# annalam/seqkit

Hardware: AMD Instinct MI355X
Metric: M reads/s demultiplex (150bp, 96 barcodes) at 1/8 GPUs; % HBM roofline (higher is better)
Workload: dtype u8

## Files before the change

### seqkit_amd/build.py

```python
from __future__ import annotations

import os
import shutil
import subprocess
import sys

ROOT = os.path.dirname(os.path.abspath(__file__))
REPO = os.path.dirname(ROOT)
CSRC = os.path.join(ROOT, "csrc")
LIBDIR = os.path.join(ROOT, "lib")
BINDIR = os.path.join(ROOT, "bin")
LIB_PATH = os.path.join(LIBDIR, "libseqkit_hip.so")

HIP_SOURCES = ["sk_kernels.hip", "sk_census.hip", "sk_inflate.hip", "sk_deflate.hip", "sk_bamtext.hip", "sk_bamwrite.hip", "sk_bamminimize.hip", "sk_bammarkdup.hip", "sk_bamsubsample.hip", "sk_bammerge.hip", "sk_bamcoverage.hip", "sk_bampair.hip", "sk_bamtarget.hip", "sk_capi.hip", "sk_bamfile.cpp", "sk_bamfile_reads.cpp", "sk_bamfile_out.cpp", "sk_bamfile_coverage.cpp", "sk_lut.cpp"]
HIP_DEPS = HIP_SOURCES + ["sk_internal.h", "sk_lut.h", "sk_bamblock.h", "sk_bamfmt.h", "sk_bamfile.h", "sk_passmem.h", os.path.join(REPO, "include", "seqkit_hip.h")]
HIP_FLAGS = ["--offload-arch=gfx950", "-O3", "-std=c++17", "-fPIC", "-shared", "-Wall", "-Wno-unused-function"]


def library_inputs_digest() -> str:
    import hashlib
    h = hashlib.sha256()
    h.update(" ".join(HIP_FLAGS).encode())
    for d in HIP_DEPS:
        p = d if os.path.isabs(d) else os.path.join(CSRC, d)
        with open(p, "rb") as f:
            h.update(os.path.basename(p).encode() + b"\0" + f.read())
    return h.hexdigest()[:16]


def _hipcc() -> str:
    for cand in (os.environ.get("HIPCC"), shutil.which("hipcc"), "/opt/rocm/bin/hipcc"):
        if cand and os.path.exists(cand):
            return cand
    raise RuntimeError("hipcc not found: the gfx950 library cannot be built")


def _stale(target: str, deps: list[str]) -> bool:
    if not os.path.exists(target):
        return True
    t = os.path.getmtime(target)
    for d in deps:
        p = d if os.path.isabs(d) else os.path.join(CSRC, d)
        if os.path.exists(p) and os.path.getmtime(p) > t:
            return True
    return False


def _run(cmd: list[str], cwd: str) -> None:
    r = subprocess.run(cmd, cwd=cwd, stdout=subprocess.PIPE, stderr=subprocess.STDOUT, text=True)
    if r.returncode != 0:
        sys.stderr.write(r.stdout)
        raise RuntimeError("build failed: " + " ".join(cmd))


def build_library(force: bool = False, verbose: bool = False) -> str:
    os.makedirs(LIBDIR, exist_ok=True)
    if force or _stale(LIB_PATH, HIP_DEPS):
        cmd = [_hipcc()] + HIP_FLAGS + ["-o", LIB_PATH] + HIP_SOURCES + ["-ldl", "-lz", "-pthread"]
        if verbose:
            cmd.append("-Rpass-analysis=kernel-resource-usage")
        _run(cmd, CSRC)
    return LIB_PATH


def build_hosts(force: bool = False) -> list[str]:
    os.makedirs(BINDIR, exist_ok=True)
    out = []
    for name, srcs, libs in (("fasta", ["host_common.cpp", "host_inflate.cpp", "fasta_main.cpp", "fasta_text.cpp"], ["-lz", "-ldl"]),
                             ("sam", ["host_common.cpp", "host_inflate.cpp", "sam_main.cpp"], ["-lz", "-ldl"])):
        if not all(os.path.exists(os.path.join(CSRC, s)) for s in srcs):
            continue
        target = os.path.join(BINDIR, name)
        deps = srcs + ["host_common.h", "sam_pairing.h", "sk_bamfmt.h", os.path.join(REPO, "include", "seqkit_hip.h"), LIB_PATH]
        if force or _stale(target, deps):
            cmd = ["g++", "-O2", "-std=c++17", "-Wall", "-Wextra", "-pthread", "-I", os.path.join(REPO, "include"),
                   "-o", target] + srcs + ["-L", LIBDIR, "-lseqkit_hip", "-Wl,-rpath,$ORIGIN/../lib"] + libs
            _run(cmd, CSRC)
        out.append(target)
    return out


def build_all(force: bool = False) -> None:
    build_library(force=force)
    build_hosts(force=force)


if __name__ == "__main__":
    build_all(force="--force" in sys.argv)
    print(LIB_PATH)
```

### seqkit_amd/csrc/sk_kernels.hip

```cpp
#include "sk_internal.h"

#include <cstdlib>
#include <mutex>
#include <vector>

namespace sk {

#ifndef SK_STRAGGLER_FROM
#define SK_STRAGGLER_FROM 6
#endif
#ifndef SK_STRAGGLER_ROWS
#define SK_STRAGGLER_ROWS 8
#endif
#ifndef SK_STRAGGLER_LEFT
#define SK_STRAGGLER_LEFT 6
#endif

typedef uint32_t u32;
typedef __attribute__((ext_vector_type(4))) uint32_t u32x4;
typedef __attribute__((ext_vector_type(2))) uint32_t u32x2;

typedef const __attribute__((address_space(4))) uint32_t *const_u32_ptr;

constexpr u32 kLo7 = 0x7f7f7f7fu;
constexpr u32 kHi1 = 0x80808080u;

QualConsts make_qual_consts(int m)
{
	QualConsts q{};
	q.min_baseq = m;
	q.cl2 = 0; q.c72 = 0;
	if (m == 0) { q.mode = 0; return q; }
	int t2;
	if (33 + m <= 255) { q.mode = 1; t2 = 33 + m; }
	else if (33 + m == 256) { q.mode = 3; t2 = 1; }
	else { q.mode = 4; t2 = 33 + m - 256; }
	int c2 = 256 - t2;
	q.cl2 = (u32)(c2 & 0x7f) * 0x01010101u;
	q.c72 = (c2 & 0x80) ? kHi1 : 0u;
	if (q.mode == 1 && !(c2 & 0x80)) q.mode = 2;
	return q;
}

template <int MODE>
__device__ __forceinline__ u32 lowq_flags(u32 q, u32 ql, u32 t1, u32 cl2)
{
	if (MODE == 0) return 0u;
	u32 g1 = q | t1;
	if (MODE == 3) return g1;
	u32 t2 = ql + cl2;
	u32 g2 = (MODE == 2) ? (q & t2) : (q | t2);
	if (MODE == 4) return g1 | ~g2;
	return g1 & ~g2;
}

__device__ __forceinline__ u32 mask_select(u32 s, u32 F)
{
	u32 sel = ((F >> 5) & 0x04040404u) | 0x03020100u;
	return __builtin_amdgcn_perm(0x4e4e4e4eu, s, sel);
}

__device__ __forceinline__ u32 sub33(u32 q, u32 t1) { return t1 ^ (~q & kHi1); }

template <int MODE>
__device__ __forceinline__ void mask_dword4(const u32x4 &q, const u32x4 &s, u32 cl2, u32x4 &out, u32x4 &vq)
{
#pragma unroll
	for (int i = 0; i < 4; i++) {
		u32 ql = q[i] & kLo7;
		u32 t1 = ql + 0x5f5f5f5fu;
		vq[i] = sub33(q[i], t1);
		out[i] = mask_select(s[i], lowq_flags<MODE>(q[i], ql, t1, cl2));
	}
}

#ifndef SK_NT
#define SK_NT 3
#endif
__device__ __forceinline__ u32x4 stream_load(const uint8_t *p)
{
#if SK_NT & 1
	return __builtin_nontemporal_load(reinterpret_cast<const u32x4 *>(p));
#else
	return *reinterpret_cast<const u32x4 *>(p);
#endif
}
__device__ __forceinline__ void stream_store(uint8_t *p, const u32x4 &v)
{
#if SK_NT & 2
	__builtin_nontemporal_store(v, reinterpret_cast<u32x4 *>(p));
#else
	*reinterpret_cast<u32x4 *>(p) = v;
#endif
}

__device__ __forceinline__ u32x4 load_tail(const uint8_t *p, int valid)
{
	u32x4 v = {0u, 0u, 0u, 0u};
	for (int b = 0; b < valid; b++) v[b >> 2] |= (u32)p[b] << (8 * (b & 3));
	return v;
}
__device__ __forceinline__ void store_tail(uint8_t *p, const u32x4 &v, int valid)
{
	for (int b = 0; b < valid; b++) p[b] = (uint8_t)(v[b >> 2] >> (8 * (b & 3)));
}

template <int MODE>
__global__ __launch_bounds__(256) void mask_flat_kernel(const uint8_t *__restrict__ seq, const uint8_t *__restrict__ qual,
                                                        uint8_t *__restrict__ out, int64_t bytes, u32 cl2)
{
#ifndef SK_MASK_UNROLL
#define SK_MASK_UNROLL 4
#endif
	constexpr int kUnroll = SK_MASK_UNROLL;
	const int64_t nchunk = (bytes + 15) >> 4;
	const int64_t nspan = (nchunk + 256 * kUnroll - 1) / (256 * kUnroll);
	for (int64_t sp = blockIdx.x; sp < nspan; sp += gridDim.x) {
		const int64_t c0 = sp * (256 * kUnroll) + (threadIdx.x >> 6) * (64 * kUnroll) + (threadIdx.x & 63);
		if ((sp + 1) * (256 * kUnroll) * 16 <= bytes) {
			u32x4 q[kUnroll], sv[kUnroll];
#pragma unroll
			for (int k = 0; k < kUnroll; k++) {
				const int64_t off = (c0 + k * 64) << 4;
				q[k] = stream_load(qual + off);
				sv[k] = stream_load(seq + off);
			}
#pragma unroll
			for (int k = 0; k < kUnroll; k++) {
				u32x4 o, vq;
				mask_dword4<MODE>(q[k], sv[k], cl2, o, vq);
				stream_store(out + ((c0 + k * 64) << 4), o);
			}
		} else {
			for (int k = 0; k < kUnroll; k++) {
				const int64_t c = c0 + k * 64;
				if (c >= nchunk) break;
				const int64_t off = c << 4;
				u32x4 q, s, o, vq;
				if (off + 16 <= bytes) {
					q = *reinterpret_cast<const u32x4 *>(qual + off);
					s = *reinterpret_cast<const u32x4 *>(seq + off);
					mask_dword4<MODE>(q, s, cl2, o, vq);
					*reinterpret_cast<u32x4 *>(out + off) = o;
				} else {
					int valid = (int)(bytes - off);
					q = load_tail(qual + off, valid);
					s = load_tail(seq + off, valid);
					mask_dword4<MODE>(q, s, cl2, o, vq);
					store_tail(out + off, o, valid);
				}
			}
		}
	}
// ... 1934 lines not shown
			u32x4 e4 = {0u, 0u, 0u, 0u}, mt4 = e4, mp4 = e4, tl4 = e4;
			if (a.single_end) e4 = *reinterpret_cast<const u32x4 *>(a.end_pos + r0);
			else {
				mt4 = *reinterpret_cast<const u32x4 *>(a.mtid + r0);
				mp4 = *reinterpret_cast<const u32x4 *>(a.mpos + r0);
				tl4 = *reinterpret_cast<const u32x4 *>(a.tlen + r0);
			}
#pragma unroll
			for (int u = 0; u < kCountIlp; u++) {
				fl[u] = (f2[u >> 1] >> (16 * (u & 1))) & 0xffffu;
				mq[u] = (m4 >> (8 * u)) & 0xffu;
				posv[u] = (int32_t)p4[u]; tidv[u] = (int32_t)t4[u];
				mtidv[u] = (int32_t)mt4[u]; mposv[u] = (int32_t)mp4[u]; tlenv[u] = (int32_t)tl4[u]; endv[u] = (int32_t)e4[u];
			}
		} else {
#pragma unroll
			for (int u = 0; u < kCountIlp; u++) {
				const int64_t rc = r0 + u < a.n ? r0 + u : r0;
				fl[u] = a.flag[rc]; mq[u] = a.mapq[rc]; posv[u] = a.pos[rc]; tidv[u] = a.tid[rc];
				endv[u] = a.single_end ? a.end_pos[rc] : 0;
				mtidv[u] = a.single_end ? 0 : a.mtid[rc]; mposv[u] = a.single_end ? 0 : a.mpos[rc]; tlenv[u] = a.single_end ? 0 : a.tlen[rc];
			}
		}
		u32 start[kCountIlp], end[kCountIlp];
		int lo[kCountIlp], b[kCountIlp], e[kCountIlp];
#pragma unroll
		for (int u = 0; u < kCountIlp; u++) {
			const u32 f = fl[u];
			bool ok = r0 + u < a.n;
			ok = ok && !(f & (0x4u | 0x400u | 0x100u | 0x800u));
			ok = ok && mq[u] >= a.min_mapq;
			const int32_t pos = posv[u], tid = tidv[u];
			u32 st = (u32)pos, en;
			if (a.single_end) {
				en = (u32)endv[u];
			} else {
				ok = ok && (f & 0x1u) && !(f & 0x8u);
				ok = ok && tid == mtidv[u];
				const int32_t mpos = mposv[u];
				ok = ok && !(pos > mpos || (pos == mpos && !(f & 0x40u)));
				const int32_t tl = tlenv[u];
				const u32 ins = tl < 0 ? 0u - (u32)tl : (u32)tl;
				ok = ok && ins >= 20u;
				en = st + ins;
			}
			ok = ok && en - st <= a.max_frag_len;
			if (a.center) { st += (en - st) / 2u; en = st + 1u; }
			ok = ok && tid >= 0 && tid < a.n_chr;
			const int tc = ok ? tid : 0;
			lo[u] = a.chr_off[tc];
			b[u] = lo[u];
			e[u] = ok ? a.chr_off[tc + 1] : lo[u];
			start[u] = st;
			end[u] = en;
		}
		int hi_prev = -1;
#pragma unroll
		for (int u = 0; u < kCountIlp; u++) {
			const int hi = e[u];
			if (u > 0 && lo[u] == lo[u - 1] && hi == hi_prev && hi > lo[u]) b[u] = region_gallop(a.rstart, lo[u], hi, b[u - 1], end[u]);
			else b[u] = region_lower_bound(a.rstart, lo[u], hi, end[u]);
			hi_prev = hi;
		}
#pragma unroll
		for (int u = 0; u < kCountIlp; u++) {
			for (int i = b[u] - 1; i >= lo[u]; i--) {
				if (a.rpmax[i] <= start[u]) break;
				if (a.rend[i] > start[u]) atomicAdd(&a.counts[a.ridx[i]], 1u);
			}
		}
	}
}

hipError_t launch_bam_count(const CountArgs &a, int n_cu, hipStream_t st)
{
	if (a.n <= 0) return hipSuccess;
	const int64_t want = (a.n + 256 * kCountIlp - 1) / (256 * kCountIlp);
	const int grid = (int)(want < (int64_t)n_cu * 8 ? want : (int64_t)n_cu * 8);
	uintptr_t bits = (uintptr_t)a.flag | (uintptr_t)a.mapq | (uintptr_t)a.pos | (uintptr_t)a.tid;
	bits |= a.single_end ? (uintptr_t)a.end_pos : ((uintptr_t)a.mtid | (uintptr_t)a.mpos | (uintptr_t)a.tlen);
	if ((bits & 15u) == 0) bam_count_kernel<true><<<grid, 256, 0, st>>>(a);
	else bam_count_kernel<false><<<grid, 256, 0, st>>>(a);
	return hipGetLastError();
}

__device__ __forceinline__ u32 zero_bytes(u32 x)
{
	return ~(((x & 0x7F7F7F7Fu) + 0x7F7F7F7Fu) | x | 0x7F7F7F7Fu);
}

__device__ __forceinline__ void gc_dword(u32 w, u32 &gc, u32 &non_n)
{
	const u32 up = w & 0xDFDFDFDFu;
	gc += (u32)__popc(zero_bytes(up ^ 0x43434343u) | zero_bytes(up ^ 0x47474747u));
	non_n += 4u - (u32)__popc(zero_bytes(up ^ 0x4E4E4E4Eu));
}

__device__ __forceinline__ void gc_byte(u32 b, u32 &gc, u32 &non_n)
{
	const u32 up = b & 0xDFu;
	gc += (up == 0x43u || up == 0x47u) ? 1u : 0u;
	non_n += (up != 0x4Eu) ? 1u : 0u;
}

__global__ __launch_bounds__(256) void gc_count_kernel(const uint8_t *__restrict__ genome, const int64_t *__restrict__ seg_start,
                                                       const int32_t *__restrict__ seg_len, const int32_t *__restrict__ seg_region, int64_t nseg,
                                                       unsigned long long *__restrict__ out )
{
	const int lane = threadIdx.x & 63;
	const int64_t wave = ((int64_t)blockIdx.x * blockDim.x + threadIdx.x) >> 6, nwaves = ((int64_t)gridDim.x * blockDim.x) >> 6;
	for (int64_t s = wave; s < nseg; s += nwaves) {
		const uint8_t *p = genome + seg_start[s];
		const int n = seg_len[s];
		u32 gc = 0, non_n = 0;
		int head = (int)((16 - ((uintptr_t)p & 15)) & 15);
		if (head > n) head = n;
		if (lane < head) gc_byte(p[lane], gc, non_n);
		const int body = (n - head) & ~15;
		const u32x4 *v = reinterpret_cast<const u32x4 *>(p + head);
		const int nchunk = body >> 4;
		int i = lane;
		for (; i + 192 < nchunk; i += 256) {
			u32x4 w[4];
#pragma unroll
			for (int k = 0; k < 4; k++) w[k] = stream_load(reinterpret_cast<const uint8_t *>(v + i + 64 * k));
#pragma unroll
			for (int k = 0; k < 4; k++) { gc_dword(w[k][0], gc, non_n); gc_dword(w[k][1], gc, non_n); gc_dword(w[k][2], gc, non_n); gc_dword(w[k][3], gc, non_n); }
		}
		for (; i < nchunk; i += 64) {
			const u32x4 w = stream_load(reinterpret_cast<const uint8_t *>(v + i));
			gc_dword(w[0], gc, non_n); gc_dword(w[1], gc, non_n); gc_dword(w[2], gc, non_n); gc_dword(w[3], gc, non_n);
		}
		const int tail0 = head + body;
		if (tail0 + lane < n) gc_byte(p[tail0 + lane], gc, non_n);
		for (int o = 32; o > 0; o >>= 1) { gc += __shfl_xor(gc, o); non_n += __shfl_xor(non_n, o); }
		if (lane == 0) {
			const int r = seg_region[s];
			if (gc) atomicAdd(&out[2 * r], (unsigned long long)gc);
			if (non_n) atomicAdd(&out[2 * r + 1], (unsigned long long)non_n);
		}
	}
}

hipError_t launch_gc_count(const uint8_t *genome, const int64_t *seg_start, const int32_t *seg_len, const int32_t *seg_region, int64_t nseg,
                           unsigned long long *out, int n_cu, hipStream_t st)
{
	if (nseg <= 0) return hipSuccess;
	const int64_t want = (nseg + 3) / 4;
	const int grid = (int)(want < (int64_t)n_cu * 8 ? want : (int64_t)n_cu * 8);
	gc_count_kernel<<<grid, 256, 0, st>>>(genome, seg_start, seg_len, seg_region, nseg, out);
	return hipGetLastError();
}

constexpr u32 kN4 = 0x4E4E4E4Eu;

__device__ __forceinline__ u32 bases_from_codes(u32 nib, bool complement)
{
	const u32 lo = complement ? 0x4E47544Eu : 0x4E43414Eu;
	const u32 hi = complement ? 0x4E4E4E43u : 0x4E4E4E47u;
	const u32 lo8 = complement ? 0x4E4E4E41u : 0x4E4E4E54u;
	const u32 sel = nib & 0x07070707u;
	const u32 r_low = __builtin_amdgcn_perm(hi, lo, sel);
	const u32 r_high = __builtin_amdgcn_perm(kN4, lo8, sel);
	const u32 is_high = ((nib >> 3) & 0x01010101u) * 0xFFu;
	return (r_high & is_high) | (r_low & ~is_high);
}

template <bool SMALL_M>
__device__ __forceinline__ u32 bytes_below(u32 q, u32 m4)
{
	const u32 d = (q | kHi1) - (m4 & ~kHi1);
	const u32 lt = SMALL_M ? (~(q | d) & kHi1) : (((~q & m4) | (~(q ^ m4) & ~d)) & kHi1);
	return (lt >> 7) * 0xFFu;
}

__device__ __forceinline__ u32 spread_nibbles(u32 h)
{
	u32 x = (h | (h << 8)) & 0x00FF00FFu;
	return (x | (x << 4)) & 0x0F0F0F0Fu;
}

#ifndef SK_SEQ_UNROLL
#define SK_SEQ_UNROLL 1
#endif
constexpr int kSeqUnroll = SK_SEQ_UNROLL;
template <bool SMALL_M>
__global__ __launch_bounds__(256) void bam_sequence8_kernel(const uint8_t *__restrict__ seq4, int seq4_stride, const uint8_t *__restrict__ qual,
                                                            int stride, const uint16_t *__restrict__ len, const uint16_t *__restrict__ flag,
                                                            int64_t n, u32 m4, u32 inv_upr, uint8_t *__restrict__ out)
{
	__shared__ u32 row_info[64];
	const int upr = (stride + 7) >> 3;
	const bool half_tail = (stride & 7) != 0;
	const int64_t ntiles = (n + 63) / 64;
	for (int64_t t = blockIdx.x; t < ntiles; t += gridDim.x) {
		const int64_t row0 = t * 64;
		const int rows = (int)((n - row0) < 64 ? (n - row0) : 64);
		__syncthreads();
		if ((int)threadIdx.x < rows) {
			const int64_t r = row0 + threadIdx.x;
			const u32 l = len ? (u32)len[r] : (u32)stride;
			row_info[threadIdx.x] = l | (((u32)flag[r] >> 4) & 1u) << 16;
		}
		__syncthreads();
		const rsrc_t rq = make_rsrc(qual, row0 * (int64_t)stride, rows * stride);
		const rsrc_t rs = make_rsrc(seq4, row0 * (int64_t)seq4_stride, rows * seq4_stride);
		const rsrc_t ro = make_rsrc(out, row0 * (int64_t)stride, rows * stride);
		const u32 total = (u32)rows * (u32)upr;
		for (u32 e = threadIdx.x; e < total; e += blockDim.x * kSeqUnroll) {
			u32 rlv[kSeqUnroll], w0v[kSeqUnroll];
			int jv[kSeqUnroll], s0v[kSeqUnroll];
			bool revv[kSeqUnroll];
			u32x2 w12v[kSeqUnroll], ddv[kSeqUnroll];
#pragma unroll
			for (int u = 0; u < kSeqUnroll; u++) {
				const u32 eu = e + (u32)u * blockDim.x;
				const u32 ec = eu < total ? eu : total - 1;
				const u32 rl = inv_upr ? __umulhi(ec, inv_upr) : ec / (u32)upr;
				const int j = (int)(ec - rl * (u32)upr);
				const u32 info = row_info[rl];
				const int l = (int)(info & 0xFFFFu);
				const bool rev = (info >> 16) != 0u;
				int s0 = rev ? l - 8 - 8 * j : 8 * j;
				if (s0 < -8) s0 = -8;
				const int qrow = (int)rl * stride, qd = s0 >> 2;
				w0v[u] = __builtin_amdgcn_raw_buffer_load_b32(rq, qrow + 4 * (qd < 0 ? 0 : qd), 0, 0);
				w12v[u] = __builtin_amdgcn_raw_buffer_load_b64(rq, qrow + 4 * (qd + 1 < 0 ? 0 : qd + 1), 0, 0);
				const int sd = (s0 >> 1) >> 2;
				ddv[u] = __builtin_amdgcn_raw_buffer_load_b64(rs, (int)rl * seq4_stride + 4 * (sd < 0 ? 0 : sd), 0, 0);
				rlv[u] = rl; jv[u] = j; s0v[u] = s0; revv[u] = rev;
			}
#pragma unroll
			for (int u = 0; u < kSeqUnroll; u++) {
				const int s0 = s0v[u];
				const bool rev = revv[u];
				const int qd = s0 >> 2;
				const u32 sh = (u32)s0 & 3u;
				const u32 w0 = w0v[u], w1 = w12v[u][0], w2 = qd + 1 < 0 ? w12v[u][0] : w12v[u][1];
				const u32 qa = __builtin_amdgcn_alignbyte(w1, w0, sh), qb = __builtin_amdgcn_alignbyte(w2, w1, sh);
				const int a = s0 >> 1, sd = a >> 2;
				const u32 d0 = ddv[u][0], d1 = sd < 0 ? ddv[u][0] : ddv[u][1];
				const u32 b03 = __builtin_amdgcn_alignbyte(d1, d0, (u32)a & 3u);
				const u32 b4 = __builtin_amdgcn_alignbyte(0u, d1, (u32)a & 3u) & 0xFFu;
				const u32 be = __builtin_bswap32(b03);
				const u32 n8 = (s0 & 1) ? ((be << 4) | (b4 >> 4)) : be;
				const u32 c_first = spread_nibbles(n8 >> 16), c_last = spread_nibbles(n8 & 0xFFFFu);
				u32 q_lo, q_hi, n_lo, n_hi;
				if (rev) {
					q_lo = __builtin_amdgcn_perm(0u, qb, 0x00010203u); q_hi = __builtin_amdgcn_perm(0u, qa, 0x00010203u);
					n_lo = c_last; n_hi = c_first;
				} else {
					q_lo = qa; q_hi = qb;
					n_lo = __builtin_amdgcn_perm(0u, c_first, 0x00010203u); n_hi = __builtin_amdgcn_perm(0u, c_last, 0x00010203u);
				}
				const u32 lo_low = bytes_below<SMALL_M>(q_lo, m4), hi_low = bytes_below<SMALL_M>(q_hi, m4);
				u32x2 o;
				o[0] = (kN4 & lo_low) | (bases_from_codes(n_lo, rev) & ~lo_low);
				o[1] = (kN4 & hi_low) | (bases_from_codes(n_hi, rev) & ~hi_low);
				if (e + (u32)u * blockDim.x < total) {
					if (half_tail && jv[u] == upr - 1) __builtin_amdgcn_raw_buffer_store_b32(o[0], ro, (int)rlv[u] * stride + 8 * jv[u], 0, 0);
					else __builtin_amdgcn_raw_buffer_store_b64(o, ro, (int)rlv[u] * stride + 8 * jv[u], 0, 0);
				}
			}
		}
	}
}

#ifndef SK_SEQ_TWO
#define SK_SEQ_TWO 0
#endif
template <bool SMALL_M, int NQ, int ROWS>
__global__ __launch_bounds__(256, ROWS == 64 ? 2 : 4) void bam_sequence_tile_kernel(const uint8_t *__restrict__ seq4, int seq4_stride, const uint8_t *__restrict__ qual,
                                                                   int stride, const uint16_t *__restrict__ len, const uint16_t *__restrict__ flag,
                                                                   int64_t n, u32 m4, u32 inv_upr, uint8_t *__restrict__ out)
{
	constexpr int NS = (NQ + 1) / 2;
	constexpr int kSlot = (NQ + NS) * 1024 + 256;
	constexpr int kMaxU = NQ * 2;
	static_assert(ROWS == 64 || ROWS == 32, "a tile is one or half a row per lane");
	const int lane = threadIdx.x & 63;
	const int wave = __builtin_amdgcn_readfirstlane(threadIdx.x >> 6);
	uint8_t *img = sk_smem + wave * kSlot;
	uint8_t *simg = img + NQ * 1024;
	u32 *info = reinterpret_cast<u32 *>(img + (NQ + NS) * 1024);
	const int upr = (stride + 7) >> 3;
	const bool half_tail = (stride & 4) != 0;
	const int64_t ntiles = (n + ROWS - 1) / ROWS;
	const int64_t tstep = (int64_t)gridDim.x * 4;
	auto fetch = [&](int64_t t, u32x4 (&rq)[NQ], u32x4 (&rs)[NS], u32 &rinfo) {
		const int rows = t < ntiles ? (int)((n - t * ROWS) < ROWS ? (n - t * ROWS) : ROWS) : 0;
		const int64_t row0 = rows ? t * ROWS : 0;
		const rsrc_t dq = make_rsrc(qual, row0 * (int64_t)stride, rows * stride), ds = make_rsrc(seq4, row0 * (int64_t)seq4_stride, (rows * seq4_stride + 3) & ~3);
#pragma unroll
		for (int c = 0; c < NQ; c++) rq[c] = __builtin_amdgcn_raw_buffer_load_b128(dq, c * 1024 + lane * 16, 0, kAuxStream);
#pragma unroll
		for (int c = 0; c < NS; c++) rs[c] = __builtin_amdgcn_raw_buffer_load_b128(ds, c * 1024 + lane * 16, 0, kAuxStream);
		const u32 lv = (u32)(unsigned short)__builtin_amdgcn_raw_buffer_load_b16(make_rsrc(len, row0 * 2, rows * 2), lane * 2, 0, 0);
		const u32 fv = (u32)(unsigned short)__builtin_amdgcn_raw_buffer_load_b16(make_rsrc(flag, row0 * 2, rows * 2), lane * 2, 0, 0);
		rinfo = (len ? lv : (u32)stride) | ((fv >> 4) & 1u) << 16;
	};
	auto process = [&](int64_t t, int ahead, u32x4 (&rq)[NQ], u32x4 (&rs)[NS], u32 &rinfo) {
		const int64_t row0 = t * ROWS;
		const int rows = (int)((n - row0) < ROWS ? (n - row0) : ROWS);
		const u32 units = (u32)(ROWS * upr);
#pragma unroll
		for (int c = 0; c < NQ; c++) *reinterpret_cast<u32x4 *>(img + c * 1024 + lane * 16) = rq[c];
#pragma unroll
		for (int c = 0; c < NS; c++) *reinterpret_cast<u32x4 *>(simg + c * 1024 + lane * 16) = rs[c];
		info[lane] = rinfo;
		wave_lds_fence();
		fetch(t + ahead * tstep, rq, rs, rinfo);
		u32x2 ov[kMaxU];
#pragma unroll
		for (int i = 0; i < kMaxU; i++) {
			ov[i][0] = ov[i][1] = 0u;
			if (64u * (u32)i < units) {
				const u32 ee = (u32)lane + 64u * (u32)i;
				const u32 e = ee < units ? ee : units - 1u;
				const u32 rl = inv_upr ? __umulhi(e, inv_upr) : e / (u32)upr;
				const int j = (int)(e - rl * (u32)upr);
				const u32 inf = info[rl];
				const int l = (int)(inf & 0xFFFFu);
				const bool rev = (inf >> 16) != 0u;
				int s0 = rev ? l - 8 - 8 * j : 8 * j;
				if (s0 < -8) s0 = -8;
				const int qrow = (int)rl * stride, qd = s0 >> 2;
				const u32 *qw = reinterpret_cast<const u32 *>(img + qrow);
				const u32 w0 = qw[qd < 0 ? 0 : qd], w1 = qw[qd + 1 < 0 ? 0 : qd + 1], w2 = qw[qd + 2 < 0 ? 0 : qd + 2];
				const u32 sh = (u32)s0 & 3u;
				const u32 qa = __builtin_amdgcn_alignbyte(w1, w0, sh), qb = __builtin_amdgcn_alignbyte(w2, w1, sh);
				const int a = s0 >> 1, sd = a >> 2;
				const u32 *sw = reinterpret_cast<const u32 *>(simg + (int)rl * seq4_stride);
				const u32 d0 = sw[sd < 0 ? 0 : sd], d1 = sw[sd + 1 < 0 ? 0 : sd + 1];
				const u32 b03 = __builtin_amdgcn_alignbyte(d1, d0, (u32)a & 3u);
				const u32 b4 = __builtin_amdgcn_alignbyte(0u, d1, (u32)a & 3u) & 0xFFu;
				const u32 be = __builtin_bswap32(b03);
				const u32 n8 = (s0 & 1) ? ((be << 4) | (b4 >> 4)) : be;
				const u32 c_first = spread_nibbles(n8 >> 16), c_last = spread_nibbles(n8 & 0xFFFFu);
				u32 q_lo, q_hi, n_lo, n_hi;
				if (rev) {
					q_lo = __builtin_amdgcn_perm(0u, qb, 0x00010203u); q_hi = __builtin_amdgcn_perm(0u, qa, 0x00010203u);
					n_lo = c_last; n_hi = c_first;
				} else {
					q_lo = qa; q_hi = qb;
					n_lo = __builtin_amdgcn_perm(0u, c_first, 0x00010203u); n_hi = __builtin_amdgcn_perm(0u, c_last, 0x00010203u);
				}
				const u32 lo_low = bytes_below<SMALL_M>(q_lo, m4), hi_low = bytes_below<SMALL_M>(q_hi, m4);
				ov[i][0] = (kN4 & lo_low) | (bases_from_codes(n_lo, rev) & ~lo_low);
				ov[i][1] = (kN4 & hi_low) | (bases_from_codes(n_hi, rev) & ~hi_low);
			}
		}
		wave_lds_fence();
		if (!half_tail) {
#pragma unroll
			for (int i = 0; i < kMaxU; i++)
				if ((u32)lane + 64u * (u32)i < units) *reinterpret_cast<u32x2 *>(img + 8 * (lane + 64 * i)) = ov[i];
		} else {
#pragma unroll
			for (int i = 0; i < kMaxU; i++) {
				const u32 e = (u32)lane + 64u * (u32)i;
				if (e < units) {
					const u32 rl = inv_upr ? __umulhi(e, inv_upr) : e / (u32)upr;
					const int j = (int)(e - rl * (u32)upr);
					u32 *dst = reinterpret_cast<u32 *>(img + (int)rl * stride + 8 * j);
					dst[0] = ov[i][0];
					if (j != upr - 1) dst[1] = ov[i][1];
				}
			}
		}
		wave_lds_fence();
		const rsrc_t dout = make_rsrc(out, row0 * (int64_t)stride, rows * stride);
#pragma unroll
		for (int c = 0; c < NQ; c++) {
			const u32x4 v = *reinterpret_cast<const u32x4 *>(img + c * 1024 + lane * 16);
			__builtin_amdgcn_raw_buffer_store_b128(v, dout, c * 1024 + lane * 16, 0, kAuxStreamSt);
		}
		wave_lds_fence();
	};
	int64_t t = (int64_t)blockIdx.x * 4 + wave;
#if SK_SEQ_TWO
	u32x4 rqa[NQ], rsa[NS], rqb[NQ], rsb[NS];
	u32 ia = 0u, ib = 0u;
	fetch(t, rqa, rsa, ia);
	fetch(t + tstep, rqb, rsb, ib);
	for (; t < ntiles; t += 2 * tstep) {
		process(t, 2, rqa, rsa, ia);
		if (t + tstep < ntiles) process(t + tstep, 2, rqb, rsb, ib);
	}
#else
	u32x4 rq[NQ], rs[NS];
	u32 rinfo = 0u;
	fetch(t, rq, rs, rinfo);
	for (; t < ntiles; t += tstep) process(t, 1, rq, rs, rinfo);
#endif
}

hipError_t launch_bam_sequence(const uint8_t *seq4, int seq4_stride, const uint8_t *qual, int stride, const uint16_t *len, const uint16_t *flag,
                               int64_t n, int min_baseq, uint8_t *out, int n_cu, hipStream_t st)
{
	if (n <= 0) return hipSuccess;
	const int64_t ntiles = (n + 63) / 64;
	static const int wgs = getenv("SK_SEQ_WGS") ? atoi(getenv("SK_SEQ_WGS")) : 8;
	const int grid = (int)(ntiles < (int64_t)n_cu * wgs ? ntiles : (int64_t)n_cu * wgs);
	const u32 m4 = (u32)(min_baseq & 0xFF) * 0x01010101u;
	const u32 upr = ((u32)stride + 7u) >> 3;
	const u32 inv8 = (upr > 1 && upr < 8192u) ? (u32)(((1ull << 32) + upr - 1) / upr) : 0u;
	const char *env_tile = getenv("SK_SEQ_TILE");
	const bool env_no_tile = env_tile && atoi(env_tile) == 0;
	if (!env_no_tile && (stride & 3) == 0 && stride >= 8 && 64 * stride <= 10 * 1024 && (seq4_stride & 3) == 0 && 64 * seq4_stride <= 5 * 1024 &&
	    ((uintptr_t)seq4 & 15) == 0 && ((uintptr_t)qual & 15) == 0 && ((uintptr_t)out & 15) == 0) {
		const bool small = (min_baseq & 0xFF) < 128;
		constexpr int kNQ = 10;
		const int lds = 4 * ((kNQ + (kNQ + 1) / 2) * 1024 + 256);
		const void *fn = small ? reinterpret_cast<const void *>(bam_sequence_tile_kernel<true, kNQ, 64>) : reinterpret_cast<const void *>(bam_sequence_tile_kernel<false, kNQ, 64>);
		hipError_t e = hipFuncSetAttribute(fn, hipFuncAttributeMaxDynamicSharedMemorySize, lds);
		if (e != hipSuccess) return e;
		const int64_t want = (ntiles + 3) / 4;
		const int g2 = (int)(want < (int64_t)n_cu * 2 ? want : (int64_t)n_cu * 2);
		void *kargs[] = {(void *)&seq4, (void *)&seq4_stride, (void *)&qual, (void *)&stride, (void *)&len, (void *)&flag, (void *)&n, (void *)&m4, (void *)&inv8, (void *)&out};
		return hipLaunchKernel(fn, dim3((unsigned)g2), dim3(256), kargs, (size_t)lds, st);
	}
	if ((min_baseq & 0xFF) < 128)
		bam_sequence8_kernel<true><<<grid, 256, 0, st>>>(seq4, seq4_stride, qual, stride, len, flag, n, m4, inv8, out);
	else
		bam_sequence8_kernel<false><<<grid, 256, 0, st>>>(seq4, seq4_stride, qual, stride, len, flag, n, m4, inv8, out);
	return hipGetLastError();
}

hipError_t launch_bam_fragments(const uint16_t *flag, const int32_t *tid, const int32_t *mtid, const int32_t *tlen, int64_t n,
                                int64_t min_size, int64_t max_size, uint8_t *keep_bits, unsigned long long *kept, int n_cu, hipStream_t st)
{
	if (n <= 0) return hipSuccess;
	const int64_t lo = min_size < 0 ? 0 : min_size, hi = max_size > 0x80000000ll ? 0x80000000ll : max_size;
	const u32 ulo = lo > 0x80000000ll ? 0xffffffffu : (u32)lo, uhi = hi < 0 ? 0u : (u32)hi;
	const bool empty = hi < 0 || lo > hi;
	int64_t want = (n + 2047) / 2048;
	static const int wgs = getenv("SK_BAM_WGS") ? atoi(getenv("SK_BAM_WGS")) : 2;
	int grid = (int)(want < (int64_t)n_cu * wgs ? want : (int64_t)n_cu * wgs);
	bam_fragments_kernel<<<grid, 256, 0, st>>>(flag, tid, mtid, tlen, n, empty ? 1u : ulo, empty ? 0u : uhi, keep_bits, kept);
	return hipGetLastError();
}

hipError_t launch_bam_flag_tlen(const uint16_t *flag, const int32_t *tid, const int32_t *mtid, const int32_t *tlen,
                                int64_t n, int32_t max_frag, unsigned long long *out, int want_counters, int want_hist,
                                int n_cu, hipStream_t st)
{
	if (n <= 0) return hipSuccess;
	int64_t bins = want_hist ? (int64_t)max_frag + 1 : 0;
	int lds_bins = (int)(bins < 15360 ? bins : 15360);
	const bool aligned = (((uintptr_t)flag | (want_hist ? ((uintptr_t)tid | (uintptr_t)mtid | (uintptr_t)tlen) : 0)) & 15u) == 0;
	if (aligned) {
		int64_t want = (n + 2047) / 2048;
		static const int wgs = getenv("SK_BAM_WGS") ? atoi(getenv("SK_BAM_WGS")) : 2;
		int grid = (int)(want < (int64_t)n_cu * wgs ? want : (int64_t)n_cu * wgs);
		bam_flag_tlen_kernel<<<grid, 256, lds_bins * 4, st>>>(flag, tid, mtid, tlen, n, max_frag, out, want_counters, want_hist, lds_bins);
	} else {
		int64_t want = (n + 255) / 256;
		int grid = (int)(want < (int64_t)n_cu * 4 ? want : (int64_t)n_cu * 4);
		bam_flag_tlen_scalar_kernel<<<grid, 256, lds_bins * 4, st>>>(flag, tid, mtid, tlen, n, max_frag, out, want_counters, want_hist, lds_bins);
	}
	return hipGetLastError();
}

}
```

Baseline: 6717.

## Decode sequence tiles row-per-lane with precomputed per-row permute selectors

Adds a BY_ROW variant of the tile kernel in which each lane decodes one whole row from LDS. Per-row constants (perm selectors, shifts) are computed once, and the per-unit row/column division and info lookups are dropped. The variant is chosen when the stride's power-of-two factor keeps LDS bank conflicts low. The decode math is also rewritten to use byte-permute selects instead of mask/blend arithmetic, and moved into a shared header. This shortens the ALU path but changes the LDS access pattern and may raise register pressure.

```diff
diff --git a/seqkit_amd/build.py b/seqkit_amd/build.py
--- a/seqkit_amd/build.py
+++ b/seqkit_amd/build.py
@@ -13,7 +13,7 @@
 LIB_PATH = os.path.join(LIBDIR, "libseqkit_hip.so")
 
 HIP_SOURCES = ["sk_kernels.hip", "sk_census.hip", "sk_inflate.hip", "sk_deflate.hip", "sk_bamtext.hip", "sk_bamwrite.hip", "sk_bamminimize.hip", "sk_bammarkdup.hip", "sk_bamsubsample.hip", "sk_bammerge.hip", "sk_bamcoverage.hip", "sk_bampair.hip", "sk_bamtarget.hip", "sk_capi.hip", "sk_bamfile.cpp", "sk_bamfile_reads.cpp", "sk_bamfile_out.cpp", "sk_bamfile_coverage.cpp", "sk_lut.cpp"]
-HIP_DEPS = HIP_SOURCES + ["sk_internal.h", "sk_lut.h", "sk_bamblock.h", "sk_bamfmt.h", "sk_bamfile.h", "sk_passmem.h", os.path.join(REPO, "include", "seqkit_hip.h")]
+HIP_DEPS = HIP_SOURCES + ["sk_internal.h", "sk_lut.h", "sk_bamblock.h", "sk_bamfmt.h", "sk_bamfile.h", "sk_passmem.h", "sk_seqdecode.h", os.path.join(REPO, "include", "seqkit_hip.h")]
 HIP_FLAGS = ["--offload-arch=gfx950", "-O3", "-std=c++17", "-fPIC", "-shared", "-Wall", "-Wno-unused-function"]
 
 
diff --git a/seqkit_amd/csrc/sk_kernels.hip b/seqkit_amd/csrc/sk_kernels.hip
--- a/seqkit_amd/csrc/sk_kernels.hip
+++ b/seqkit_amd/csrc/sk_kernels.hip
@@ -1,4 +1,5 @@
 #include "sk_internal.h"
+#include "sk_seqdecode.h"
 
 #include <cstdlib>
 #include <mutex>
@@ -2239,34 +2240,6 @@
 	return hipGetLastError();
 }
 
-constexpr u32 kN4 = 0x4E4E4E4Eu;
-
-__device__ __forceinline__ u32 bases_from_codes(u32 nib, bool complement)
-{
-	const u32 lo = complement ? 0x4E47544Eu : 0x4E43414Eu;
-	const u32 hi = complement ? 0x4E4E4E43u : 0x4E4E4E47u;
-	const u32 lo8 = complement ? 0x4E4E4E41u : 0x4E4E4E54u;
-	const u32 sel = nib & 0x07070707u;
-	const u32 r_low = __builtin_amdgcn_perm(hi, lo, sel);
-	const u32 r_high = __builtin_amdgcn_perm(kN4, lo8, sel);
-	const u32 is_high = ((nib >> 3) & 0x01010101u) * 0xFFu;
-	return (r_high & is_high) | (r_low & ~is_high);
-}
-
-template <bool SMALL_M>
-__device__ __forceinline__ u32 bytes_below(u32 q, u32 m4)
-{
-	const u32 d = (q | kHi1) - (m4 & ~kHi1);
-	const u32 lt = SMALL_M ? (~(q | d) & kHi1) : (((~q & m4) | (~(q ^ m4) & ~d)) & kHi1);
-	return (lt >> 7) * 0xFFu;
-}
-
-__device__ __forceinline__ u32 spread_nibbles(u32 h)
-{
-	u32 x = (h | (h << 8)) & 0x00FF00FFu;
-	return (x | (x << 4)) & 0x0F0F0F0Fu;
-}
-
 #ifndef SK_SEQ_UNROLL
 #define SK_SEQ_UNROLL 1
 #endif
@@ -2295,7 +2268,7 @@
 		const rsrc_t ro = make_rsrc(out, row0 * (int64_t)stride, rows * stride);
 		const u32 total = (u32)rows * (u32)upr;
 		for (u32 e = threadIdx.x; e < total; e += blockDim.x * kSeqUnroll) {
-			u32 rlv[kSeqUnroll], w0v[kSeqUnroll];
+			u32 rlv[kSeqUnroll], w0v[kSeqUnroll], lv[kSeqUnroll];
 			int jv[kSeqUnroll], s0v[kSeqUnroll];
 			bool revv[kSeqUnroll];
 			u32x2 w12v[kSeqUnroll], ddv[kSeqUnroll];
@@ -2315,35 +2288,19 @@
 				w12v[u] = __builtin_amdgcn_raw_buffer_load_b64(rq, qrow + 4 * (qd + 1 < 0 ? 0 : qd + 1), 0, 0);
 				const int sd = (s0 >> 1) >> 2;
 				ddv[u] = __builtin_amdgcn_raw_buffer_load_b64(rs, (int)rl * seq4_stride + 4 * (sd < 0 ? 0 : sd), 0, 0);
-				rlv[u] = rl; jv[u] = j; s0v[u] = s0; revv[u] = rev;
+				rlv[u] = rl; jv[u] = j; s0v[u] = s0; revv[u] = rev; lv[u] = (u32)l;
 			}
 #pragma unroll
 			for (int u = 0; u < kSeqUnroll; u++) {
 				const int s0 = s0v[u];
 				const bool rev = revv[u];
-				const int qd = s0 >> 2;
-				const u32 sh = (u32)s0 & 3u;
-				const u32 w0 = w0v[u], w1 = w12v[u][0], w2 = qd + 1 < 0 ? w12v[u][0] : w12v[u][1];
-				const u32 qa = __builtin_amdgcn_alignbyte(w1, w0, sh), qb = __builtin_amdgcn_alignbyte(w2, w1, sh);
-				const int a = s0 >> 1, sd = a >> 2;
-				const u32 d0 = ddv[u][0], d1 = sd < 0 ? ddv[u][0] : ddv[u][1];
-				const u32 b03 = __builtin_amdgcn_alignbyte(d1, d0, (u32)a & 3u);
-				const u32 b4 = __builtin_amdgcn_alignbyte(0u, d1, (u32)a & 3u) & 0xFFu;
-				const u32 be = __builtin_bswap32(b03);
-				const u32 n8 = (s0 & 1) ? ((be << 4) | (b4 >> 4)) : be;
-				const u32 c_first = spread_nibbles(n8 >> 16), c_last = spread_nibbles(n8 & 0xFFFFu);
-				u32 q_lo, q_hi, n_lo, n_hi;
-				if (rev) {
-					q_lo = __builtin_amdgcn_perm(0u, qb, 0x00010203u); q_hi = __builtin_amdgcn_perm(0u, qa, 0x00010203u);
-					n_lo = c_last; n_hi = c_first;
-				} else {
-					q_lo = qa; q_hi = qb;
-					n_lo = __builtin_amdgcn_perm(0u, c_first, 0x00010203u); n_hi = __builtin_amdgcn_perm(0u, c_last, 0x00010203u);
-				}
-				const u32 lo_low = bytes_below<SMALL_M>(q_lo, m4), hi_low = bytes_below<SMALL_M>(q_hi, m4);
+				const int qd = s0 >> 2, sd = (s0 >> 1) >> 2;
+				const u32 w2 = qd + 1 < 0 ? w12v[u][0] : w12v[u][1];
+				const u32 d1 = sd < 0 ? ddv[u][0] : ddv[u][1];
 				u32x2 o;
-				o[0] = (kN4 & lo_low) | (bases_from_codes(n_lo, rev) & ~lo_low);
-				o[1] = (kN4 & hi_low) | (bases_from_codes(n_hi, rev) & ~hi_low);
+				u32 o0, o1;
+				seqdec::unit<SMALL_M>(w0v[u], w12v[u][0], w2, ddv[u][0], d1, seqdec::row_consts(lv[u], rev), m4, o0, o1);
+				o[0] = o0; o[1] = o1;
 				if (e + (u32)u * blockDim.x < total) {
 					if (half_tail && jv[u] == upr - 1) __builtin_amdgcn_raw_buffer_store_b32(o[0], ro, (int)rlv[u] * stride + 8 * jv[u], 0, 0);
 					else __builtin_amdgcn_raw_buffer_store_b64(o, ro, (int)rlv[u] * stride + 8 * jv[u], 0, 0);
@@ -2353,10 +2310,7 @@
 	}
 }
 
-#ifndef SK_SEQ_TWO
-#define SK_SEQ_TWO 0
-#endif
-template <bool SMALL_M, int NQ, int ROWS>
+template <bool SMALL_M, int NQ, int ROWS, bool BY_ROW>
 __global__ __launch_bounds__(256, ROWS == 64 ? 2 : 4) void bam_sequence_tile_kernel(const uint8_t *__restrict__ seq4, int seq4_stride, const uint8_t *__restrict__ qual,
                                                                    int stride, const uint16_t *__restrict__ len, const uint16_t *__restrict__ flag,
                                                                    int64_t n, u32 m4, u32 inv_upr, uint8_t *__restrict__ out)
@@ -2365,6 +2319,7 @@
 	constexpr int kSlot = (NQ + NS) * 1024 + 256;
 	constexpr int kMaxU = NQ * 2;
 	static_assert(ROWS == 64 || ROWS == 32, "a tile is one or half a row per lane");
+	static_assert(!BY_ROW || ROWS == 64, "lane r owns row r");
 	const int lane = threadIdx.x & 63;
 	const int wave = __builtin_amdgcn_readfirstlane(threadIdx.x >> 6);
 	uint8_t *img = sk_smem + wave * kSlot;
@@ -2394,64 +2349,53 @@
 		for (int c = 0; c < NQ; c++) *reinterpret_cast<u32x4 *>(img + c * 1024 + lane * 16) = rq[c];
 #pragma unroll
 		for (int c = 0; c < NS; c++) *reinterpret_cast<u32x4 *>(simg + c * 1024 + lane * 16) = rs[c];
-		info[lane] = rinfo;
+		if constexpr (!BY_ROW) info[lane] = rinfo;
+		const u32 my_info = rinfo;
 		wave_lds_fence();
 		fetch(t + ahead * tstep, rq, rs, rinfo);
-		u32x2 ov[kMaxU];
-#pragma unroll
-		for (int i = 0; i < kMaxU; i++) {
-			ov[i][0] = ov[i][1] = 0u;
-			if (64u * (u32)i < units) {
-				const u32 ee = (u32)lane + 64u * (u32)i;
-				const u32 e = ee < units ? ee : units - 1u;
-				const u32 rl = inv_upr ? __umulhi(e, inv_upr) : e / (u32)upr;
-				const int j = (int)(e - rl * (u32)upr);
-				const u32 inf = info[rl];
-				const int l = (int)(inf & 0xFFFFu);
-				const bool rev = (inf >> 16) != 0u;
-				int s0 = rev ? l - 8 - 8 * j : 8 * j;
-				if (s0 < -8) s0 = -8;
-				const int qrow = (int)rl * stride, qd = s0 >> 2;
-				const u32 *qw = reinterpret_cast<const u32 *>(img + qrow);
-				const u32 w0 = qw[qd < 0 ? 0 : qd], w1 = qw[qd + 1 < 0 ? 0 : qd + 1], w2 = qw[qd + 2 < 0 ? 0 : qd + 2];
-				const u32 sh = (u32)s0 & 3u;
-				const u32 qa = __builtin_amdgcn_alignbyte(w1, w0, sh), qb = __builtin_amdgcn_alignbyte(w2, w1, sh);
-				const int a = s0 >> 1, sd = a >> 2;
-				const u32 *sw = reinterpret_cast<const u32 *>(simg + (int)rl * seq4_stride);
-				const u32 d0 = sw[sd < 0 ? 0 : sd], d1 = sw[sd + 1 < 0 ? 0 : sd + 1];
-				const u32 b03 = __builtin_amdgcn_alignbyte(d1, d0, (u32)a & 3u);
-				const u32 b4 = __builtin_amdgcn_alignbyte(0u, d1, (u32)a & 3u) & 0xFFu;
-				const u32 be = __builtin_bswap32(b03);
-				const u32 n8 = (s0 & 1) ? ((be << 4) | (b4 >> 4)) : be;
-				const u32 c_first = spread_nibbles(n8 >> 16), c_last = spread_nibbles(n8 & 0xFFFFu);
-				u32 q_lo, q_hi, n_lo, n_hi;
-				if (rev) {
-					q_lo = __builtin_amdgcn_perm(0u, qb, 0x00010203u); q_hi = __builtin_amdgcn_perm(0u, qa, 0x00010203u);
-					n_lo = c_last; n_hi = c_first;
-				} else {
-					q_lo = qa; q_hi = qb;
-					n_lo = __builtin_amdgcn_perm(0u, c_first, 0x00010203u); n_hi = __builtin_amdgcn_perm(0u, c_last, 0x00010203u);
-				}
-				const u32 lo_low = bytes_below<SMALL_M>(q_lo, m4), hi_low = bytes_below<SMALL_M>(q_hi, m4);
-				ov[i][0] = (kN4 & lo_low) | (bases_from_codes(n_lo, rev) & ~lo_low);
-				ov[i][1] = (kN4 & hi_low) | (bases_from_codes(n_hi, rev) & ~hi_low);
-			}
-		}
-		wave_lds_fence();
-		if (!half_tail) {
-#pragma unroll
-			for (int i = 0; i < kMaxU; i++)
-				if ((u32)lane + 64u * (u32)i < units) *reinterpret_cast<u32x2 *>(img + 8 * (lane + 64 * i)) = ov[i];
+		const auto ldq = [&](u32 at) { return *reinterpret_cast<const u32 *>(img + at); };
+		const auto lds = [&](u32 at) { return *reinterpret_cast<const u32 *>(simg + at); };
+		if constexpr (BY_ROW) {
+			typedef __attribute__((address_space(3))) u32 lds_u32;
+			const u32 qrow = (u32)(uintptr_t)(__attribute__((address_space(3))) uint8_t *)img + (u32)(lane * stride);
+			const u32 srow = (u32)(uintptr_t)(__attribute__((address_space(3))) uint8_t *)simg + (u32)(lane * seq4_stride);
+			const auto ld = [](u32 at) { return *(const lds_u32 *)(uintptr_t)at; };
+			int upr_t = upr;
+			asm volatile("" : "+s"(upr_t));
+			seqdec::RowUnits<kMaxU> ru;
+			seqdec::decode_row<SMALL_M, kMaxU>(my_info, stride, upr_t, qrow, srow, ld, ld, m4, ru);
+			seqdec::store_row<kMaxU>(ru, upr_t, half_tail, qrow, [](u32 at, u32 v) { *(lds_u32 *)(uintptr_t)at = v; });
 		} else {
+			u32x2 ov[kMaxU];
 #pragma unroll
 			for (int i = 0; i < kMaxU; i++) {
-				const u32 e = (u32)lane + 64u * (u32)i;
-				if (e < units) {
+				ov[i][0] = ov[i][1] = 0u;
+				if (64u * (u32)i < units) {
+					const u32 ee = (u32)lane + 64u * (u32)i;
+					const u32 e = ee < units ? ee : units - 1u;
 					const u32 rl = inv_upr ? __umulhi(e, inv_upr) : e / (u32)upr;
 					const int j = (int)(e - rl * (u32)upr);
-					u32 *dst = reinterpret_cast<u32 *>(img + (int)rl * stride + 8 * j);
-					dst[0] = ov[i][0];
-					if (j != upr - 1) dst[1] = ov[i][1];
+					u32 o0, o1;
+					seqdec::unit_of_row<SMALL_M>(info[rl], j, rl * (u32)stride, rl * (u32)seq4_stride, ldq, lds, m4, o0, o1);
+					ov[i][0] = o0; ov[i][1] = o1;
+				}
+			}
+			wave_lds_fence();
+			if (!half_tail) {
+#pragma unroll
+				for (int i = 0; i < kMaxU; i++)
+					if ((u32)lane + 64u * (u32)i < units) *reinterpret_cast<u32x2 *>(img + 8 * (lane + 64 * i)) = ov[i];
+			} else {
+#pragma unroll
+				for (int i = 0; i < kMaxU; i++) {
+					const u32 e = (u32)lane + 64u * (u32)i;
+					if (e < units) {
+						const u32 rl = inv_upr ? __umulhi(e, inv_upr) : e / (u32)upr;
+						const int j = (int)(e - rl * (u32)upr);
+						u32 *dst = reinterpret_cast<u32 *>(img + (int)rl * stride + 8 * j);
+						dst[0] = ov[i][0];
+						if (j != upr - 1) dst[1] = ov[i][1];
+					}
 				}
 			}
 		}
@@ -2465,21 +2409,10 @@
 		wave_lds_fence();
 	};
 	int64_t t = (int64_t)blockIdx.x * 4 + wave;
-#if SK_SEQ_TWO
-	u32x4 rqa[NQ], rsa[NS], rqb[NQ], rsb[NS];
-	u32 ia = 0u, ib = 0u;
-	fetch(t, rqa, rsa, ia);
-	fetch(t + tstep, rqb, rsb, ib);
-	for (; t < ntiles; t += 2 * tstep) {
-		process(t, 2, rqa, rsa, ia);
-		if (t + tstep < ntiles) process(t + tstep, 2, rqb, rsb, ib);
-	}
-#else
 	u32x4 rq[NQ], rs[NS];
 	u32 rinfo = 0u;
 	fetch(t, rq, rs, rinfo);
 	for (; t < ntiles; t += tstep) process(t, 1, rq, rs, rinfo);
-#endif
 }
 
 hipError_t launch_bam_sequence(const uint8_t *seq4, int seq4_stride, const uint8_t *qual, int stride, const uint16_t *len, const uint16_t *flag,
@@ -2499,7 +2432,10 @@
 		const bool small = (min_baseq & 0xFF) < 128;
 		constexpr int kNQ = 10;
 		const int lds = 4 * ((kNQ + (kNQ + 1) / 2) * 1024 + 256);
-		const void *fn = small ? reinterpret_cast<const void *>(bam_sequence_tile_kernel<true, kNQ, 64>) : reinterpret_cast<const void *>(bam_sequence_tile_kernel<false, kNQ, 64>);
+		const u32 p4 = (u32)stride >> 2;
+		const bool by_row = (p4 & (0u - p4)) <= 4u;
+		const void *fn = by_row ? (small ? reinterpret_cast<const void *>(bam_sequence_tile_kernel<true, kNQ, 64, true>) : reinterpret_cast<const void *>(bam_sequence_tile_kernel<false, kNQ, 64, true>))
+		                        : (small ? reinterpret_cast<const void *>(bam_sequence_tile_kernel<true, kNQ, 64, false>) : reinterpret_cast<const void *>(bam_sequence_tile_kernel<false, kNQ, 64, false>));
 		hipError_t e = hipFuncSetAttribute(fn, hipFuncAttributeMaxDynamicSharedMemorySize, lds);
 		if (e != hipSuccess) return e;
 		const int64_t want = (ntiles + 3) / 4;
diff --git a/seqkit_amd/csrc/sk_seqdecode.h b/seqkit_amd/csrc/sk_seqdecode.h
--- /dev/null
+++ b/seqkit_amd/csrc/sk_seqdecode.h
@@ -0,0 +1,164 @@
+#pragma once
+#include <stdint.h>
+
+#ifndef SK_HD
+#if defined(__HIPCC__)
+#define SK_HD __host__ __device__
+#else
+#define SK_HD
+#endif
+#endif
+
+namespace sk {
+namespace seqdec {
+
+typedef uint32_t u32;
+
+constexpr u32 kN4 = 0x4E4E4E4Eu;
+constexpr u32 kTop = 0x80808080u;
+
+SK_HD inline u32 perm8(u32 hi, u32 lo, u32 sel)
+{
+#if defined(__HIP_DEVICE_COMPILE__)
+	return __builtin_amdgcn_perm(hi, lo, sel);
+#else
+	u32 out = 0;
+	for (int k = 0; k < 4; k++) {
+		const u32 q = (sel >> (8 * k)) & 7u;
+		out |= ((q < 4 ? lo >> (8 * q) : hi >> (8 * (q - 4))) & 0xFFu) << (8 * k);
+	}
+	return out;
+#endif
+}
+SK_HD inline u32 alignbyte(u32 hi, u32 lo, u32 sh)
+{
+#if defined(__HIP_DEVICE_COMPILE__)
+	return __builtin_amdgcn_alignbyte(hi, lo, sh);
+#else
+	sh &= 3u;
+	return sh ? (lo >> (8 * sh)) | (hi << (32 - 8 * sh)) : lo;
+#endif
+}
+
+SK_HD inline u32 bases_from_codes(u32 nib, u32 t_lo, u32 t_hi, u32 t_lo8)
+{
+	const u32 sel = nib & 0x07070707u;
+	const u32 r_low = perm8(t_hi, t_lo, sel);
+	const u32 r_high = perm8(kN4, t_lo8, sel);
+	return perm8(r_high, r_low, ((nib >> 1) & 0x04040404u) | 0x03020100u);
+}
+
+template <bool SMALL_M>
+SK_HD inline u32 bytes_below(u32 q, u32 m4)
+{
+	const u32 d = (q | kTop) - (m4 & ~kTop);
+	return SMALL_M ? (~(q | d) & kTop) : (((~q & m4) | (~(q ^ m4) & ~d)) & kTop);
+}
+SK_HD inline u32 mask_low(u32 bases, u32 below) { return perm8(kN4, bases, (below >> 5) | 0x03020100u); }
+
+struct Row {
+	u32 t_lo, t_hi, t_lo8;
+	u32 sel_qlo, sel_qhi;
+	u32 sel_nlo, sel_nhi;
+	u32 qsh, bsh;
+	u32 nsh, nmask;
+};
+SK_HD inline Row row_consts(u32 l, bool rev)
+{
+	Row r;
+	r.t_lo = rev ? 0x4E47544Eu : 0x4E43414Eu;
+	r.t_hi = rev ? 0x4E4E4E43u : 0x4E4E4E47u;
+	r.t_lo8 = rev ? 0x4E4E4E41u : 0x4E4E4E54u;
+	r.sel_qlo = rev ? 0x04050607u : 0x03020100u;
+	r.sel_qhi = rev ? 0x00010203u : 0x07060504u;
+	r.sel_nlo = rev ? 0x05010400u : 0x02060307u;
+	r.sel_nhi = rev ? 0x07030602u : 0x00040105u;
+	r.qsh = rev ? l & 3u : 0u;
+	r.bsh = rev ? (l >> 1) & 3u : 0u;
+	const bool odd = rev && (l & 1u);
+	r.nsh = odd ? 4u : 0u;
+	r.nmask = odd ? 0xFu : 0u;
+	return r;
+}
+
+template <bool SMALL_M>
+SK_HD inline void unit(u32 w0, u32 w1, u32 w2, u32 d0, u32 d1, const Row &r, u32 m4, u32 &o0, u32 &o1)
+{
+	const u32 qa = alignbyte(w1, w0, r.qsh), qb = alignbyte(w2, w1, r.qsh);
+	const u32 b03 = alignbyte(d1, d0, r.bsh);
+	const u32 b4 = alignbyte(0u, d1, r.bsh);
+	const u32 be = __builtin_bswap32(b03);
+	const u32 n8 = (be << r.nsh) | ((b4 >> 4) & r.nmask);
+	const u32 c_1st = (n8 >> 4) & 0x0F0F0F0Fu, c_2nd = n8 & 0x0F0F0F0Fu;
+	const u32 q_lo = perm8(qb, qa, r.sel_qlo), q_hi = perm8(qb, qa, r.sel_qhi);
+	const u32 n_lo = perm8(c_1st, c_2nd, r.sel_nlo), n_hi = perm8(c_1st, c_2nd, r.sel_nhi);
+	const u32 lo_low = bytes_below<SMALL_M>(q_lo, m4), hi_low = bytes_below<SMALL_M>(q_hi, m4);
+	o0 = mask_low(bases_from_codes(n_lo, r.t_lo, r.t_hi, r.t_lo8), lo_low);
+	o1 = mask_low(bases_from_codes(n_hi, r.t_lo, r.t_hi, r.t_lo8), hi_low);
+}
+
+template <bool SMALL_M, class LdQ, class LdS>
+SK_HD inline void unit_of_row(u32 info, int j, u32 qrow, u32 srow, const LdQ &ldq, const LdS &lds, u32 m4, u32 &o0, u32 &o1)
+{
+	const int l = (int)(info & 0xFFFFu);
+	const bool rev = (info >> 16) != 0u;
+	int s0 = rev ? l - 8 - 8 * j : 8 * j;
+	if (s0 < -8) s0 = -8;
+	const int qd = s0 >> 2, sd = (s0 >> 1) >> 2;
+	const u32 w0 = ldq(qrow + 4u * (u32)(qd < 0 ? 0 : qd)), w1 = ldq(qrow + 4u * (u32)(qd + 1 < 0 ? 0 : qd + 1)), w2 = ldq(qrow + 4u * (u32)(qd + 2 < 0 ? 0 : qd + 2));
+	const u32 d0 = lds(srow + 4u * (u32)(sd < 0 ? 0 : sd)), d1 = lds(srow + 4u * (u32)(sd + 1 < 0 ? 0 : sd + 1));
+	unit<SMALL_M>(w0, w1, w2, d0, d1, row_consts((u32)l, rev), m4, o0, o1);
+}
+
+template <int MAXU>
+struct RowUnits {
+	u32 ov[MAXU][2];
+	u32 fix[2];
+	int jfix;
+};
+template <bool SMALL_M, int MAXU, class LdQ, class LdS>
+SK_HD inline void decode_row(u32 info, int stride, int upr, u32 qrow, u32 srow, const LdQ &ldq, const LdS &lds, u32 m4, RowUnits<MAXU> &u)
+{
+	const u32 l0 = info & 0xFFFFu;
+	const u32 l = l0 < (u32)stride ? l0 : (u32)stride;
+	const bool rev = (info >> 16) != 0u;
+	const Row r = row_consts(l, rev);
+	const int sd0 = rev ? ((int)l - 8) >> 3 : 0;
+	const int sdir = rev ? -4 : 4;
+	int sa = (int)srow + 4 * (sd0 < 0 ? 0 : sd0);
+	const u32 qk = qrow + (rev ? (l & 4u) : 0u) - 2u * srow;
+#if defined(__HIP_DEVICE_COMPILE__)
+#pragma unroll
+#endif
+	for (int j = 0; j < MAXU; j++) {
+		u.ov[j][0] = u.ov[j][1] = 0u;
+		if (j < upr) {
+			const u32 qa = ((u32)sa << 1) + qk;
+			unit<SMALL_M>(ldq(qa), ldq(qa + 4u), ldq(qa + 8u), lds((u32)sa), lds((u32)sa + 4u), r, m4, u.ov[j][0], u.ov[j][1]);
+			sa += sdir;
+			sa = sa < (int)srow ? (int)srow : sa;
+		}
+	}
+	const u32 q0 = ldq(qrow), q1 = ldq(qrow + 4u), c0 = lds(srow);
+	unit<SMALL_M>(q0, q0, (l & 4u) ? q1 : q0, c0, c0, r, m4, u.fix[0], u.fix[1]);
+	u.jfix = (rev && (l & 7u)) ? (int)((l - 1u) >> 3) : -1;
+}
+template <int MAXU, class St>
+SK_HD inline void store_row(const RowUnits<MAXU> &u, int upr, bool half_tail, u32 orow, const St &st)
+{
+#if defined(__HIP_DEVICE_COMPILE__)
+#pragma unroll
+#endif
+	for (int j = 0; j < MAXU; j++)
+		if (j < upr) {
+			if (half_tail && j == upr - 1) st(orow + 8u * (u32)j, u.ov[j][0]);
+			else { st(orow + 8u * (u32)j, u.ov[j][0]); st(orow + 8u * (u32)j + 4u, u.ov[j][1]); }
+		}
+	if (u.jfix >= 0) {
+		st(orow + 8u * (u32)u.jfix, u.fix[0]);
+		if (!(half_tail && u.jfix == upr - 1)) st(orow + 8u * (u32)u.jfix + 4u, u.fix[1]);
+	}
+}
+
+}
+}
```

Result: slower. 6581 (-2.0%).
